# arendu-zz/MacaronicUserModeling

Hardware: AMD Instinct MI355X
Metric: LBP sweep iters/sec (whole node), batch=8192 graphs |X|=64 (higher is better)
Workload: dtype f64

## Files before the change

### macaronicusermodeling_amd/csrc/mlbp_lean.hip

```cpp
#include <hip/hip_runtime.h>

#include <vector>

#include "mlbp_device.h"
#include "mlbp_internal.h"

using mlbp::fail;
using namespace mlbp_dev;

namespace {

constexpr int WG = 256;

typedef double nt_d2 __attribute__((ext_vector_type(2)));
#define NT_LOAD2(p) ([&] { const nt_d2 v_ = __builtin_nontemporal_load(reinterpret_cast<const nt_d2*>(p)); return make_double2(v_.x, v_.y); }())

constexpr int GROUP_WORDS = 48;
using mlbp::UOP_VAR; using mlbp::UOP_MT; using mlbp::UOP_PSLOT_SHIFT; using mlbp::UOP_NOP; using mlbp::UOP_STORE_VF;
using mlbp::UOP_NSRC_SHIFT; using mlbp::UOP_CARRY_IN; using mlbp::UOP_CARRY_OUT;

struct LeanDev {
  const int32_t* image;
  const int32_t* readout;
  uint8_t* bail;
  int32_t n_bundles, HL, n_cprod, WL, n_ext, init, dense, keep;
};

__device__ __forceinline__ double swapadd16(double a, double b) {
  auto lo = __builtin_amdgcn_permlane16_swap((unsigned)__double2loint(a), (unsigned)__double2loint(b), false, false);
  auto hi = __builtin_amdgcn_permlane16_swap((unsigned)__double2hiint(a), (unsigned)__double2hiint(b), false, false);
  return __hiloint2double((int)hi[0], (int)lo[0]) + __hiloint2double((int)hi[1], (int)lo[1]);
}
__device__ __forceinline__ double swapadd32(double a, double b) {
  auto lo = __builtin_amdgcn_permlane32_swap((unsigned)__double2loint(a), (unsigned)__double2loint(b), false, false);
  auto hi = __builtin_amdgcn_permlane32_swap((unsigned)__double2hiint(a), (unsigned)__double2hiint(b), false, false);
  return __hiloint2double((int)hi[0], (int)lo[0]) + __hiloint2double((int)hi[1], (int)lo[1]);
}

__device__ __forceinline__ bool vote_any(bool p, int32_t* votes, int wave, int lane) {
  const int mine = __ballot(p) != 0 ? 1 : 0;
  if (lane == 0) votes[wave] = mine;
  lds_barrier();
  const int4 v = *reinterpret_cast<const int4*>(votes);
  return (v.x | v.y | v.z | v.w) != 0;
}

struct LaneGeo {
  int tm0, tm1;
  int mt;
  int red_tm;
  int red_mt;
  bool up, st_tm, st_mt, wr_tm;
};

__device__ __forceinline__ double2 lds2(const char* p) { return *reinterpret_cast<const double2*>(p); }
__device__ __forceinline__ void mul2(double2& a, const double2 b) { a.x *= b.x; a.y *= b.y; }

struct RegTable {
  const double2 (&T)[4][2];
  __device__ __forceinline__ double2 operator()(int r, int k) const { return T[r][k]; }
};
struct LdsTable {
  const double2* base;
  __device__ __forceinline__ double2 operator()(int r, int k) const { return base[(r * 2 + k) * WG]; }
};

template <bool MT, bool WIDE, typename TB>
__device__ __forceinline__ void contract(const TB T, char* wb, int u0, int s1, int s2, int s3, int s4, int vf,
                                         const LaneGeo& G, char* redA) {
  const int nsrc = (u0 >> UOP_NSRC_SHIFT) & 15;
  const bool has_vf = (u0 & UOP_STORE_VF) != 0;
  if (MT) {
    double2 ma = lds2(wb + s1 + G.mt), mb = lds2(wb + s1 + G.mt + 16);
    {
      const double2 a = lds2(wb + s2 + G.mt), b = lds2(wb + s2 + G.mt + 16);
      mul2(ma, a); mul2(mb, b);
    }
    if (nsrc > 2) {
      if (WIDE) {
        const double2 a2 = lds2(wb + s3 + G.mt), b2 = lds2(wb + s3 + G.mt + 16);
        const double2 a3 = lds2(wb + s4 + G.mt), b3 = lds2(wb + s4 + G.mt + 16);
        mul2(ma, a2); mul2(mb, b2);
        mul2(ma, a3); mul2(mb, b3);
      } else {
        mul2(ma, lds2(wb + s3 + G.mt)); mul2(mb, lds2(wb + s3 + G.mt + 16));
        if (nsrc > 3) { mul2(ma, lds2(wb + s4 + G.mt)); mul2(mb, lds2(wb + s4 + G.mt + 16)); }
      }
    }
    if (has_vf && G.st_mt) {
      *reinterpret_cast<double2*>(wb + vf + G.mt) = ma;
      *reinterpret_cast<double2*>(wb + vf + G.mt + 16) = mb;
    }
    double a00, a01, a10, a11;
    { const double2 t0 = T(0, 0), t1 = T(0, 1); a00 = ma.x * t0.x; a01 = ma.x * t0.y; a10 = ma.x * t1.x; a11 = ma.x * t1.y; }
    { const double2 t0 = T(1, 0), t1 = T(1, 1); a00 += ma.y * t0.x; a01 += ma.y * t0.y; a10 += ma.y * t1.x; a11 += ma.y * t1.y; }
    { const double2 t0 = T(2, 0), t1 = T(2, 1); a00 += mb.x * t0.x; a01 += mb.x * t0.y; a10 += mb.x * t1.x; a11 += mb.x * t1.y; }
    { const double2 t0 = T(3, 0), t1 = T(3, 1); a00 += mb.y * t0.x; a01 += mb.y * t0.y; a10 += mb.y * t1.x; a11 += mb.y * t1.y; }
    a00 += dpp_mov<0x128>(a10);
    a01 += dpp_mov<0x128>(a11);
    *reinterpret_cast<double*>(redA + G.red_mt) = swapadd32(a00, a01);
  } else {
    double2 m0 = lds2(wb + s1 + G.tm0), m1 = lds2(wb + s1 + G.tm1);
    {
      const double2 a = lds2(wb + s2 + G.tm0), b = lds2(wb + s2 + G.tm1);
      mul2(m0, a); mul2(m1, b);
    }
    if (nsrc > 2) {
      if (WIDE) {
        const double2 a2 = lds2(wb + s3 + G.tm0), b2 = lds2(wb + s3 + G.tm1);
        const double2 a3 = lds2(wb + s4 + G.tm0), b3 = lds2(wb + s4 + G.tm1);
        mul2(m0, a2); mul2(m1, b2);
        mul2(m0, a3); mul2(m1, b3);
      } else {
        mul2(m0, lds2(wb + s3 + G.tm0)); mul2(m1, lds2(wb + s3 + G.tm1));
        if (nsrc > 3) { mul2(m0, lds2(wb + s4 + G.tm0)); mul2(m1, lds2(wb + s4 + G.tm1)); }
      }
    }
    if (has_vf && G.st_tm) {
      *reinterpret_cast<double2*>(wb + vf + G.tm0) = m0;
      *reinterpret_cast<double2*>(wb + vf + G.tm1) = m1;
    }
    double v[4];
#pragma unroll
    for (int r = 0; r < 4; ++r) {
      const double2 t0 = T(r, 0), t1 = T(r, 1);
      v[r] = t0.x * m0.x;
      v[r] += t0.y * m0.y;
      v[r] += t1.x * m1.x;
      v[r] += t1.y * m1.y;
    }
    const double u0 = swapadd16(v[0], v[2]), u1 = swapadd16(v[1], v[3]);
    const double keep = G.up ? u1 : u0, send = G.up ? u0 : u1;
    double w = keep + dpp_mov<0x141>(send);
    w += dpp_mov<0xB1>(w);
    w += dpp_mov<0x4E>(w);
    *reinterpret_cast<double*>(redA + G.red_tm) = w;
  }
}

template <int NT, int NL>
__device__ __forceinline__ void front(const double2 (&tab)[NT][4][2], const double2* tl, char* wb, int u0, const int4& lo, const int4& hi,
                                      const LaneGeo& G, char* redA) {
  const int pslot = (u0 >> UOP_PSLOT_SHIFT) & 7;
#pragma unroll
  for (int p = 0; p < NT; ++p) {
    if (p == pslot) {
      if (u0 & UOP_MT) contract<true, (NT > 1)>(RegTable{tab[p]}, wb, u0, lo.y, lo.z, lo.w, hi.x, hi.y, G, redA);
      else contract<false, (NT > 1)>(RegTable{tab[p]}, wb, u0, lo.y, lo.z, lo.w, hi.x, hi.y, G, redA);
    }
  }
  if (NL > 0 && pslot >= NT) {
    const LdsTable T = {tl + (size_t)(pslot - NT) * 8 * WG};
    if (u0 & UOP_MT) contract<true, (NT > 1)>(T, wb, u0, lo.y, lo.z, lo.w, hi.x, hi.y, G, redA);
    else contract<false, (NT > 1)>(T, wb, u0, lo.y, lo.z, lo.w, hi.x, hi.y, G, redA);
  }
}

struct Src { double2 a, b; };

__device__ __forceinline__ void gather_pair(char* wb, int uA, const int4& A0, const int4& A1, int uB, const int4& B0, const int4& B1,
                                            const LaneGeo& G, Src& mA, Src& mB) {
  const bool mtA = (uA & UOP_MT) != 0, mtB = (uB & UOP_MT) != 0;
  const int a0 = mtA ? G.mt : G.tm0, a1 = mtA ? G.mt + 16 : G.tm1;
  const int b0 = mtB ? G.mt : G.tm0, b1 = mtB ? G.mt + 16 : G.tm1;
  mA.a = lds2(wb + A0.y + a0); mA.b = lds2(wb + A0.y + a1);
  mB.a = lds2(wb + B0.y + b0); mB.b = lds2(wb + B0.y + b1);
  {
    const double2 pa = lds2(wb + A0.z + a0), pb = lds2(wb + A0.z + a1);
    const double2 qa = lds2(wb + B0.z + b0), qb = lds2(wb + B0.z + b1);
    mul2(mA.a, pa); mul2(mA.b, pb);
    mul2(mB.a, qa); mul2(mB.b, qb);
  }
  if (((uA >> UOP_NSRC_SHIFT) & 15) > 2) {
    const double2 pa = lds2(wb + A0.w + a0), pb = lds2(wb + A0.w + a1);
    const double2 ra = lds2(wb + A1.x + a0), rb = lds2(wb + A1.x + a1);
    mul2(mA.a, pa); mul2(mA.b, pb);
    mul2(mA.a, ra); mul2(mA.b, rb);
  }
  if (((uB >> UOP_NSRC_SHIFT) & 15) > 2) {
    const double2 qa = lds2(wb + B0.w + b0), qb = lds2(wb + B0.w + b1);
    const double2 sa = lds2(wb + B1.x + b0), sb = lds2(wb + B1.x + b1);
    mul2(mB.a, qa); mul2(mB.b, qb);
    mul2(mB.a, sa); mul2(mB.b, sb);
  }
  if ((uA & UOP_STORE_VF) && (mtA ? G.st_mt : G.st_tm)) {
    *reinterpret_cast<double2*>(wb + A1.y + a0) = mA.a;
    *reinterpret_cast<double2*>(wb + A1.y + a1) = mA.b;
  }
  if ((uB & UOP_STORE_VF) && (mtB ? G.st_mt : G.st_tm)) {
    *reinterpret_cast<double2*>(wb + B1.y + b0) = mB.a;
    *reinterpret_cast<double2*>(wb + B1.y + b1) = mB.b;
  }
}

template <bool MT, typename TB>
__device__ __forceinline__ void contract_gathered(const TB T, const Src m, const LaneGeo& G, char* redA) {
#pragma clang fp contract(off)
  if (MT) {
    const double2 ma = m.a, mb = m.b;
    double a00, a01, a10, a11;
    { const double2 t0 = T(1, 0), t1 = T(1, 1); a00 = ma.y * t0.x; a01 = ma.y * t0.y; a10 = ma.y * t1.x; a11 = ma.y * t1.y; }
#define MLBP_ROW(mv, r) { const double2 t0 = T(r, 0), t1 = T(r, 1); a00 = __builtin_fma(mv, t0.x, a00); a01 = __builtin_fma(mv, t0.y, a01); \
                          a10 = __builtin_fma(mv, t1.x, a10); a11 = __builtin_fma(mv, t1.y, a11); }
    MLBP_ROW(ma.x, 0)
    MLBP_ROW(mb.x, 2)
    MLBP_ROW(mb.y, 3)
#undef MLBP_ROW
    a00 += dpp_mov<0x128>(a10);
    a01 += dpp_mov<0x128>(a11);
    *reinterpret_cast<double*>(redA + G.red_mt) = swapadd32(a00, a01);
  } else {
    const double2 m0 = m.a, m1 = m.b;
    double v[4];
#pragma unroll
    for (int r = 0; r < 4; ++r) {
      const double2 t0 = T(r, 0), t1 = T(r, 1);
      v[r] = t0.y * m0.y;
      v[r] = __builtin_fma(t0.x, m0.x, v[r]);
      v[r] = __builtin_fma(t1.x, m1.x, v[r]);
      v[r] = __builtin_fma(t1.y, m1.y, v[r]);
    }
    const double u0 = swapadd16(v[0], v[2]), u1 = swapadd16(v[1], v[3]);
    const double keep = G.up ? u1 : u0, send = G.up ? u0 : u1;
    double w = keep + dpp_mov<0x141>(send);
    w += dpp_mov<0xB1>(w);
    w += dpp_mov<0x4E>(w);
    *reinterpret_cast<double*>(redA + G.red_tm) = w;
  }
}

template <int NT>
__device__ __forceinline__ void front_gathered(const double2 (&tab)[NT][4][2], int u0, const Src m, const LaneGeo& G, char* redA) {
  const int pslot = (u0 >> UOP_PSLOT_SHIFT) & 7;
#pragma unroll
  for (int p = 0; p < NT; ++p) {
    if (p == pslot) {
      if (u0 & UOP_MT) contract_gathered<true>(RegTable{tab[p]}, m, G, redA);
      else contract_gathered<false>(RegTable{tab[p]}, m, G, redA);
    }
  }
}

template <int NT>
__device__ __forceinline__ void gradient_epilogue(const SweepDev& d, const GradFusedDev& gf, const double2 (&tab)[NT][4][2],
                                                  const char* wb, const int32_t* gst, double* scratch, const LaneGeo& G, int g,
                                                  int R_, int c_, int b3_) {
  constexpr int FEE = 3, FED = 6;
  const int t = threadIdx.x, lane = t & 63, wave = __builtin_amdgcn_readfirstlane(t >> 6);
  double lf[FEE] = {0.0, 0.0, 0.0};
  bool lbad = false;
  if (t < NT && t < d.P) {
    const int l0 = gf.pair_label[((size_t)g * d.P + t) * 2], l1 = gf.pair_label[((size_t)g * d.P + t) * 2 + 1];
    if ((unsigned)l0 >= 64u || (unsigned)l1 >= 64u) lbad = true;
    else {
      const double* phl = (gf.pair_phi[t] ? gf.phi_en_en_w1 : gf.phi_en_en) + ((size_t)l0 * 64 + l1) * FEE;
#pragma unroll
      for (int q = 0; q < FEE; ++q) lf[q] = phl[q];
    }
  }
  int which = 0;
  double2 W[NT][4][2];
  double* zs = scratch + 512;
  double* lfs = scratch + 544;
#pragma unroll
  for (int p = 0; p < NT; ++p) {
    double z = 0.0;
    if (p < d.P) {
      const int cs = as_const(gf.pair_c_slot)[p], rs = as_const(gf.pair_r_slot)[p];
      which |= (as_const(gf.pair_phi)[p] ? 1 : 0) << p;
      const double2 ca = lds2(wb + cs * 512 + G.mt), cb = lds2(wb + cs * 512 + G.mt + 16);
      const double2 r0 = lds2(wb + rs * 512 + G.tm0), r1 = lds2(wb + rs * 512 + G.tm1);
#pragma unroll
      for (int r = 0; r < 4; ++r) {
        const double ci = r == 0 ? ca.x : (r == 1 ? ca.y : (r == 2 ? cb.x : cb.y));
#pragma unroll
        for (int k = 0; k < 2; ++k) {
          const double2 rj = k ? r1 : r0, T = tab[p][r][k];
          W[p][r][k] = make_double2((ci * rj.x) * T.x, (ci * rj.y) * T.y);
          z += W[p][r][k].x + W[p][r][k].y;
        }
      }
      z = wave_sum(z);
      if (lane == 0) zs[wave * NT + p] = z;
    } else {
#pragma unroll
      for (int r = 0; r < 4; ++r) W[p][r][0] = W[p][r][1] = make_double2(0.0, 0.0);
    }
  }
  if (lbad) atomicExch(d.status, 1);
  if (t < NT && t < d.P) {
#pragma unroll
    for (int q = 0; q < FEE; ++q) lfs[t * FEE + q] = lf[q];
  }
  lds_barrier();
  double2 V[2][4][2];
#pragma unroll
  for (int tz = 0; tz < 2; ++tz)
#pragma unroll
    for (int r = 0; r < 4; ++r) V[tz][r][0] = V[tz][r][1] = make_double2(0.0, 0.0);
#pragma unroll
  for (int p = 0; p < NT; ++p) {
    if (p < d.P) {
      const double Z = (zs[p] + zs[NT + p]) + (zs[2 * NT + p] + zs[3 * NT + p]);
      const double inv = Z > 0.0 ? 1.0 / Z : 0.0;
      const double i0 = ((which >> p) & 1) ? 0.0 : inv, i1 = ((which >> p) & 1) ? inv : 0.0;
#pragma unroll
      for (int r = 0; r < 4; ++r)
#pragma unroll
        for (int k = 0; k < 2; ++k) {
          V[0][r][k].x += W[p][r][k].x * i0; V[0][r][k].y += W[p][r][k].y * i0;
          V[1][r][k].x += W[p][r][k].x * i1; V[1][r][k].y += W[p][r][k].y * i1;
        }
    }
  }
  double gacc[2][FEE] = {{0.0, 0.0, 0.0}, {0.0, 0.0, 0.0}};
  const int all = (1 << (d.P < NT ? d.P : NT)) - 1;
#pragma unroll
  for (int tz = 0; tz < 2; ++tz) {
    if (tz ? (which & all) == 0 : (which & all) == all) continue;
    typedef double v2d __attribute__((ext_vector_type(2)));
    typedef const v2d __attribute__((address_space(1))) * gptr2;
    const double* phi = tz ? gf.phi_en_en_w1 : gf.phi_en_en;
#pragma unroll
    for (int k = 0; k < 2; ++k) {
      const int col = 32 * (k ? 1 - b3_ : b3_) + 2 * c_;
      v2d cell[4][3];
#pragma unroll
      for (int r = 0; r < 4; ++r) {
        const gptr2 ph = (gptr2)(uintptr_t)(phi + ((size_t)(4 * R_ + r) * 64 + col) * FEE);
        cell[r][0] = ph[0]; cell[r][1] = ph[1]; cell[r][2] = ph[2];
      }
#pragma unroll
      for (int r = 0; r < 4; ++r) {
        const double w0 = V[tz][r][k].x, w1 = V[tz][r][k].y;
        gacc[tz][0] += w0 * cell[r][0].x + w1 * cell[r][1].y;
        gacc[tz][1] += w0 * cell[r][0].y + w1 * cell[r][2].x;
        gacc[tz][2] += w0 * cell[r][1].x + w1 * cell[r][2].y;
      }
    }
  }
  double gsum[FEE];
#pragma unroll
  for (int q = 0; q < FEE; ++q) gsum[q] = wave_sum(gacc[0][q] + gacc[1][q]);
  double lab_ee[FEE] = {0.0, 0.0, 0.0}, lab_ed[FED] = {0.0, 0.0, 0.0, 0.0, 0.0, 0.0};
  double exp_ee[FEE] = {0.0, 0.0, 0.0}, exp_ed[FED] = {0.0, 0.0, 0.0, 0.0, 0.0, 0.0};
  bool bad = false;
  constexpr int UB = 6;
  const int U = d.U;
  for (int u0 = wave; u0 < U; u0 += 4 * UB) {
    double b[UB], pv[UB][FED];
    int kd[UB], at[UB];
#pragma unroll
    for (int j = 0; j < UB; ++j) {
      const int u = u0 + 4 * j;
      kd[j] = -1;
      if (u < U) {
        const int kind = __builtin_amdgcn_readfirstlane(gst[2 * U + u]), obs = __builtin_amdgcn_readfirstlane(gst[3 * U + u]);
        const int lab = __builtin_amdgcn_readfirstlane(gst[4 * U + u]);
        const int cols = kind == 2 ? gf.Vde : 64;
        if ((unsigned)obs >= (unsigned)cols || (unsigned)lab >= 64u || (unsigned)kind > 2u) { bad = true; continue; }
        kd[j] = kind;
        const int slot = __builtin_amdgcn_readfirstlane(gst[u]);
        b[j] = __builtin_amdgcn_readfirstlane(gst[U + u]) ? *reinterpret_cast<const double*>(wb + slot * 512 + lane * 8) : 0.0;
        if (kind == 2) {
          const double2* ph = reinterpret_cast<const double2*>(gf.phi_en_de_t + ((size_t)obs * 64 + lane) * FED);
          at[j] = (obs * 64 + lab) * FED;
          const double2 a0 = ph[0], a1 = ph[1], a2 = ph[2];
          pv[j][0] = a0.x; pv[j][1] = a0.y; pv[j][2] = a1.x; pv[j][3] = a1.y; pv[j][4] = a2.x; pv[j][5] = a2.y;
        } else {
          typedef const double __attribute__((address_space(1))) * gptr1;
          const gptr1 ph = (gptr1)(uintptr_t)((kind ? gf.phi_en_en_w1_t : gf.phi_en_en_t) + ((size_t)obs * 64 + lane) * FEE);
          at[j] = (obs * 64 + lab) * FEE;
#pragma unroll
          for (int q = 0; q < FEE; ++q) pv[j][q] = ph[q];
        }
      }
    }
#pragma unroll
    for (int j = 0; j < UB; ++j) {
      if (kd[j] == 2) {
#pragma unroll
        for (int q = 0; q < FED; ++q) { lab_ed[q] += as_const_f64(gf.phi_en_de_t)[at[j] + q]; exp_ed[q] += b[j] * pv[j][q]; }
      } else if (kd[j] >= 0) {
        const double* base = kd[j] ? gf.phi_en_en_w1_t : gf.phi_en_en_t;
#pragma unroll
        for (int q = 0; q < FEE; ++q) { lab_ee[q] += as_const_f64(base)[at[j] + q]; exp_ee[q] += b[j] * pv[j][q]; }
      }
    }
  }
  if (bad && lane == 0) atomicExch(d.status, 1);
  constexpr int PER = FEE + FEE + FED;
  {
    double ue[FEE], ud[FED];
#pragma unroll
    for (int q = 0; q < FEE; ++q) ue[q] = lab_ee[q] - wave_sum(exp_ee[q]);
#pragma unroll
    for (int q = 0; q < FED; ++q) ud[q] = lab_ed[q] - wave_sum(exp_ed[q]);
    if (lane == 0) {
      double* o = scratch + wave * PER;
#pragma unroll
      for (int q = 0; q < FEE; ++q) o[q] = gsum[q];
#pragma unroll
      for (int q = 0; q < FEE; ++q) o[FEE + q] = ue[q];
#pragma unroll
      for (int q = 0; q < FED; ++q) o[FEE + FEE + q] = ud[q];
    }
  }
  lds_barrier();
  if (t == 0) {
    double tot[PER];
#pragma unroll
    for (int q = 0; q < PER; ++q) tot[q] = (scratch[q] + scratch[PER + q]) + (scratch[2 * PER + q] + scratch[3 * PER + q]);
    double gee[FEE];
#pragma unroll
    for (int q = 0; q < FEE; ++q) gee[q] = tot[FEE + q] - tot[q];
#pragma unroll
    for (int p = 0; p < NT; ++p) {
      if (p < d.P) {
#pragma unroll
        for (int q = 0; q < FEE; ++q) gee[q] += lfs[p * FEE + q];
      }
    }
#pragma unroll
    for (int q = 0; q < FEE; ++q) gf.grad_en_en[(size_t)g * FEE + q] = gee[q];
#pragma unroll
    for (int q = 0; q < FED; ++q) gf.grad_en_de[(size_t)g * FED + q] = tot[FEE + FEE + q];
  }
}

__device__ __forceinline__ double rescale(double r, int& bad) {
  const unsigned key = mag_key(r);
  const unsigned long long normal = __ballot(key - KEY_MIN < KEY_BAD - KEY_MIN);
  const unsigned long long wrong = __ballot(key >= KEY_BAD);
  bad |= (wrong != 0) | (normal == 0);
  const int ref = __builtin_amdgcn_readlane((int)key, normal ? __builtin_ctzll(normal) : 0);
  return __builtin_ldexp(r, 1023 - ((ref >> 20) & 0x7FF));
}

template <int NT, bool PADX, bool MULTI, int NL, bool GRAD>
__global__ __launch_bounds__(WG, (NT >= 7 ? 1 : (NT >= 4 ? 2 : 3))) void sweep_x64_lean_kernel(SweepDev d, LeanDev f, const int32_t* groups,
                                                                                             int n_groups, GradFusedDev gf) {
  int g = blockIdx.x;
  if (MULTI) {
    int lo = 0, hi = n_groups - 1;
    while (lo < hi) {
      const int mid = (lo + hi + 1) >> 1;
      if (as_const(groups)[(size_t)mid * GROUP_WORDS] <= g) lo = mid; else hi = mid - 1;
    }
    const int32_t* G = groups + (size_t)lo * GROUP_WORDS;
    const Words16 w0 = sload16(G), w1 = sload16(G + 16), w2 = sload16(G + 32);
    auto ptr = [](int32_t a, int32_t b) { return (uintptr_t)(uint32_t)a | ((uintptr_t)(uint32_t)b << 32); };
    g -= w0.w[0];
    f.image = (const int32_t*)ptr(w0.w[2], w0.w[3]); f.readout = (const int32_t*)ptr(w0.w[4], w0.w[5]);
    f.bail = (uint8_t*)ptr(w0.w[6], w0.w[7]); d.msgs = (double*)ptr(w0.w[8], w0.w[9]);
    d.marginals = (double*)ptr(w0.w[10], w0.w[11]); d.pair_tables = (const double*)ptr(w0.w[12], w0.w[13]);
    d.pair_tab = (const int32_t*)ptr(w0.w[14], w0.w[15]); d.unary_tables = (const double*)ptr(w1.w[0], w1.w[1]);
    d.unary_tab = (const int32_t*)ptr(w1.w[2], w1.w[3]); d.status = (int32_t*)ptr(w1.w[4], w1.w[5]);
    f.n_bundles = w1.w[6]; f.HL = w1.w[7]; f.n_cprod = w1.w[8]; f.WL = w1.w[9]; f.n_ext = w1.w[10];
    d.n_msgs = w1.w[11]; d.P = w1.w[12]; d.U = w1.w[13]; d.n_vars = w1.w[14]; d.n_pair_tables = w1.w[15];
    d.n_unary_tables = w2.w[0]; f.dense = w2.w[1];
  }
  extern __shared__ double lds[];
  double* work = lds;
  double* red = lds + (size_t)(d.n_msgs + f.n_ext) * 64;
  int32_t* limg = reinterpret_cast<int32_t*>(red + 4 * 256);
  double2* tl = reinterpret_cast<double2*>(limg + 16 * (f.n_bundles + 1));
  int32_t* gst = reinterpret_cast<int32_t*>(tl + (size_t)NL * 8 * WG);

  const int t = threadIdx.x, lane = t & 63, wave = __builtin_amdgcn_readfirstlane(t >> 6);
  const int X = PADX ? d.X : 64;
  const double uniform = 1.0 / (double)X;
  const double uni_l = (!PADX || lane < X) ? uniform : 0.0;
  double* gm = d.msgs + (size_t)g * d.n_msgs * X;
  const int32_t* img_hoist = f.image + 16 * (size_t)f.n_bundles;
  const int32_t* img_cprod = img_hoist + 8 * (size_t)f.HL;
  const int32_t* img_written = img_cprod + 16 * (size_t)f.n_cprod;
  int32_t* votes = reinterpret_cast<int32_t*>(red);
  constexpr bool LEAN_SYNC = !GRAD;
  constexpr bool EARLY = !GRAD;
  constexpr bool PAIR_GATHER = !GRAD && NL == 0 && NT == 3;
  static_assert(!(GRAD && PADX), "the GRAD form of phase A loads whole rows: X = 64 only");

  LaneGeo G;
  const int c_ = (lane & 7) | ((lane >> 1) & 8), b3_ = (lane >> 3) & 1, R_ = 4 * wave + (b3_ | ((lane >> 5) << 1));
  {
    const int b5 = lane >> 5, b4 = (lane >> 4) & 1, b2 = (lane >> 2) & 1;
    G.tm0 = (32 * b3_ + 2 * c_) * 8;
    G.tm1 = (32 * (1 - b3_) + 2 * c_) * 8;
    G.mt = 4 * R_ * 8;
    G.red_tm = (4 * R_ + 2 * b4 + b2) * 8;
    G.red_mt = (wave * 64 + 32 * b3_ + 2 * c_ + b5) * 8;
    G.up = b2 != 0;
    G.st_tm = wave == 0 && (lane & 0x28) == 0;
    G.st_mt = (lane & 0x17) == 0;
    G.wr_tm = (lane & 3) == 0;
  }

  if (t == 0) f.bail[g] = 0;
  int g_kind = 0, g_obs = 0, g_lab = 0;
  if (GRAD && t < d.U) {
    g_kind = gf.unary_kind[t]; g_obs = gf.unary_obs[(size_t)g * d.U + t]; g_lab = gf.unary_label[(size_t)g * d.U + t];
  }
  bool ok = true;
  const double* nowhere = reinterpret_cast<const double*>(f.image);
  constexpr int HB = 8;
  double ur[HB];
  int uslot[HB], ufac[HB];
  {
    const Words16 hl = sload16(img_hoist + wave * 2 * f.HL);
#pragma unroll
    for (int j = 0; j < HB; ++j) {
      const int u = hl.w[2 * j];
      uslot[j] = hl.w[2 * j + 1];
      ufac[j] = u;
      if (EARLY) {
        int row = -1;
        if (u >= 0) row = f.dense ? g * d.U + u : as_const(d.unary_tab)[(size_t)g * d.U + u];
        const bool in = (unsigned)row < (unsigned)d.n_unary_tables;
        if (u >= 0 && !in) ok = false;
        const double* at = in ? d.unary_tables + (size_t)row * X + (PADX ? min(lane, X - 1) : lane) : nowhere;
        ur[j] = *at;
      } else {
        ur[j] = 0.0;
        if (u >= 0) {
          const int row = f.dense ? g * d.U + u : as_const(d.unary_tab)[(size_t)g * d.U + u];
          if ((unsigned)row >= (unsigned)d.n_unary_tables) ok = false;
          else ur[j] = d.unary_tables[(size_t)row * X + lane];
        }
      }
    }
  }
  double2 tab[NT][4][2];
#pragma unroll
  for (int p = 0; p < NT; ++p) {
    if (!PADX && EARLY) {
      const int pc = p < d.P ? p : 0;
      const int ti = f.dense ? g * d.P + pc : as_const(d.pair_tab)[(size_t)g * d.P + pc];
      const bool in = (unsigned)ti < (unsigned)d.n_pair_tables;
      if (p < d.P && !in) ok = false;
      const double* T = (p < d.P && in) ? d.pair_tables + (size_t)ti * 4096 + (size_t)(4 * R_) * 64 + 2 * c_ : nowhere;
#pragma unroll
      for (int r = 0; r < 4; ++r) {
        tab[p][r][0] = NT_LOAD2(T + r * 64 + 32 * b3_);
        tab[p][r][1] = NT_LOAD2(T + r * 64 + 32 * (1 - b3_));
      }
    } else if (p < d.P) {
      const int ti = f.dense ? g * d.P + p : as_const(d.pair_tab)[(size_t)g * d.P + p];
      if ((unsigned)ti >= (unsigned)d.n_pair_tables) { ok = false; continue; }
      if (!PADX) {
        const double* T = d.pair_tables + (size_t)ti * 4096 + (size_t)(4 * R_) * 64 + 2 * c_;
#pragma unroll
        for (int r = 0; r < 4; ++r) {
          tab[p][r][0] = NT_LOAD2(T + r * 64 + 32 * b3_);
          tab[p][r][1] = NT_LOAD2(T + r * 64 + 32 * (1 - b3_));
        }
      } else {
        const double* T = d.pair_tables + (size_t)ti * X * X;
#pragma unroll
        for (int r = 0; r < 4; ++r)
#pragma unroll
          for (int k = 0; k < 2; ++k) {
            const int row = 4 * R_ + r, col = 32 * (k ? 1 - b3_ : b3_) + 2 * c_;
            tab[p][r][k].x = (row < X && col < X) ? T[(size_t)row * X + col] : 0.0;
            tab[p][r][k].y = (row < X && col + 1 < X) ? T[(size_t)row * X + col + 1] : 0.0;
          }
      }
    }
  }
#pragma unroll
  for (int p = NT; p < NT + NL; ++p) {
    if (p < d.P && !PADX) {
      const int ti = f.dense ? g * d.P + p : as_const(d.pair_tab)[(size_t)g * d.P + p];
      if ((unsigned)ti >= (unsigned)d.n_pair_tables) { ok = false; continue; }
      const double* T = d.pair_tables + (size_t)ti * 4096 + (size_t)(4 * R_) * 64 + 2 * c_;
#pragma unroll
      for (int r = 0; r < 4; ++r)
#pragma unroll
        for (int k = 0; k < 2; ++k) {
          typedef __attribute__((address_space(3))) void* lds_ptr;
          typedef const __attribute__((address_space(1))) void* glb_ptr;
          double2* dst = tl + ((p - NT) * 8 + r * 2 + k) * WG + wave * 64;
          __builtin_amdgcn_global_load_lds((glb_ptr)(T + r * 64 + 32 * (k ? 1 - b3_ : b3_)), (lds_ptr)dst, 16, 0, 0);
        }
    }
  }
  int dense_word = 0;
  bool dense_ok = true;
  if (EARLY) {
    const int i = min(t, d.P + d.U - 1);
    const int32_t* at = i < d.P ? d.pair_tab + (size_t)g * d.P + i : d.unary_tab + (size_t)g * d.U + (i - d.P);
    dense_word = *(f.dense ? at : f.image);
  } else if (f.dense) {
    for (int i = t; i < d.P + d.U; i += WG)
      dense_ok &= i < d.P ? d.pair_tab[(size_t)g * d.P + i] == g * d.P + i : d.unary_tab[(size_t)g * d.U + (i - d.P)] == g * d.U + (i - d.P);
  }
  constexpr int PW = 2;
  int32_t pre[PW];
#pragma unroll
  for (int q = 0; q < PW; ++q)
    pre[q] = EARLY ? f.image[min(t + q * WG, 16 * (f.n_bundles + 1) - 1)] : ((t + q * WG < 16 * (f.n_bundles + 1)) ? f.image[t + q * WG] : 0);
  unsigned bad_key = 0;
  {
    double2* dst = reinterpret_cast<double2*>(work);
    const int x0 = (2 * t) & 63;
    const double2 uni2 = PADX ? make_double2(x0 < X ? uniform : 0.0, x0 + 1 < X ? uniform : 0.0) : make_double2(uniform, uniform);
    if (f.init) {
      for (int i = t; i < d.n_msgs * 32; i += WG) dst[i] = uni2;
    } else if (!PADX) {
      const double2* src = reinterpret_cast<const double2*>(gm);
      for (int i = t; i < d.n_msgs * 32; i += WG) {
        const double2 v = src[i];
        bad_key = max(bad_key, max(mag_key(v.x), mag_key(v.y)));
        dst[i] = v;
      }
    } else {
      for (int i = t; i < d.n_msgs * 64; i += WG) {
        const int slot = i >> 6, x = i & 63;
        const double v = x < X ? gm[(size_t)slot * X + x] : 0.0;
        bad_key = max(bad_key, mag_key(v));
        work[i] = v;
      }
    }
    if (t < 32) dst[d.n_msgs * 32 + t] = uni2;
    if (t >= 32 && t < 64) dst[(d.n_msgs + f.n_ext - 1) * 32 + (t - 32)] = make_double2(1.0, 1.0);
  }
  lds_barrier();
#pragma unroll
  for (int j = 0; j < HB; ++j) {
    if (uslot[j] >= 0) {
      const double r = (!PADX || lane < X) ? ur[j] : 0.0;
      const double s = wave_sum(r);
      const double m = renorm(r, s, uni_l, true);
      bad_key = max(bad_key, s > 0.0 ? mag_key(m) : KEY_BAD);
      work[uslot[j] * 64 + lane] = m;
      if (GRAD && lane == 0) { gst[ufac[j]] = uslot[j]; gst[d.U + ufac[j]] = s > 0.0 ? 1 : 0; }
    }
  }
  if (GRAD && t < d.U) { gst[2 * d.U + t] = g_kind; gst[3 * d.U + t] = g_obs; gst[4 * d.U + t] = g_lab; }
  for (int j = HB; j < f.HL; ++j) {
    const const_i32p hp = as_const(img_hoist + (wave * f.HL + j) * 2);
    const int u = hp[0], slot = hp[1];
    if (u < 0) break;
    const int row = f.dense ? g * d.U + u : as_const(d.unary_tab)[(size_t)g * d.U + u];
    double r = 0.0;
    if ((unsigned)row >= (unsigned)d.n_unary_tables) ok = false;
    else if (!PADX || lane < X) r = d.unary_tables[(size_t)row * X + lane];
    const double s = wave_sum(r);
    const double m = renorm(r, s, uni_l, true);
    bad_key = max(bad_key, s > 0.0 ? mag_key(m) : KEY_BAD);
    work[slot * 64 + lane] = m;
    if (GRAD && lane == 0) { gst[u] = slot; gst[d.U + u] = s > 0.0 ? 1 : 0; }
  }
  if (LEAN_SYNC ? vote_any(!ok, votes, wave, lane) : !__syncthreads_and(ok ? 1 : 0)) {
    if (t == 0) atomicExch(d.status, 1);
    if (f.init)
      for (int i = t; i < d.n_msgs * X; i += WG) gm[i] = uniform;
    return;
  }
  for (int k = wave; k < f.n_cprod; k += 4) {
    const Words16 cl = sload16(img_cprod + 16 * k);
    double acc = uni_l;
#pragma unroll
    for (int q0 = 1; q0 < 16; q0 += 5) {
      if (cl.w[0] >= q0) {
        double m[5];
#pragma unroll
        for (int q = 0; q < 5; ++q) m[q] = work[cl.w[q0 + q] * 64 + lane];
#pragma unroll
        for (int q = 0; q < 5; ++q) acc *= m[q];
      }
    }
    bad_key = max(bad_key, mag_key(acc));
    work[(d.n_msgs + 1 + k) * 64 + lane] = acc;
  }
  auto fill_limg = [&]() {
    if (NL > 0) asm volatile("s_waitcnt vmcnt(0)" ::: "memory");
#pragma unroll
    for (int q = 0; q < PW; ++q)
      if (t + q * WG < 16 * (f.n_bundles + 1)) limg[t + q * WG] = pre[q];
    for (int i = t + PW * WG; i < 16 * (f.n_bundles + 1); i += WG) limg[i] = f.image[i];
  };
  if (LEAN_SYNC) fill_limg();
  if (LEAN_SYNC ? vote_any(bad_key >= KEY_BAD, votes + 1024, wave, lane) : __syncthreads_or(bad_key >= KEY_BAD ? 1 : 0) != 0) {
    if (t == 0) f.bail[g] = 1;
    return;
  }
  if (!LEAN_SYNC) { fill_limg(); lds_barrier(); }

  char* wb = reinterpret_cast<char*>(work);
  int parity = 0, bad = 0;
  double carry = 1.0;
  const int4* li = reinterpret_cast<const int4*>(limg);
  int4 A0 = li[0], A1 = li[1], B0 = li[2], B1 = li[3];
  for (int k = 0; k < f.n_bundles; ++k) {
    int4 nA0, nA1, nB0, nB1;
#define MLBP_FETCH_NEXT() (nA0 = li[4 * k + 4], nA1 = li[4 * k + 5], nB0 = li[4 * k + 6], nB1 = li[4 * k + 7])
    if (!PAIR_GATHER) MLBP_FETCH_NEXT();
    const int fA = __builtin_amdgcn_readfirstlane(A0.x), fB = __builtin_amdgcn_readfirstlane(B0.x);
    if (fA & UOP_VAR) {
      if (PAIR_GATHER) MLBP_FETCH_NEXT();
      const int nsrc = (fA >> UOP_NSRC_SHIFT) & 15;
      double m = work[(A0.y >> 3) + lane];
      const double m2 = work[(A0.z >> 3) + lane];
      if (fA & UOP_CARRY_IN) m *= carry;
      m *= m2;
      if (nsrc > 2) {
        const double m3 = work[(A0.w >> 3) + lane], m4 = work[(A1.x >> 3) + lane];
        m *= m3;
        m *= m4;
      }
      if (fA & UOP_CARRY_OUT) carry = m;
      else work[(A1.y >> 3) + lane] = m;
    } else {
      char* redP = reinterpret_cast<char*>(red) + parity * 4096;
      const bool two = !(fB & UOP_NOP);
      if (PAIR_GATHER) {
        Src mA, mB;
        gather_pair(wb, fA, A0, A1, fB, B0, B1, G, mA, mB);
        MLBP_FETCH_NEXT();
        front_gathered<NT>(tab, fA, mA, G, redP);
        if (two) front_gathered<NT>(tab, fB, mB, G, redP + 2048);
      } else {
        front<NT, NL>(tab, tl + t, wb, fA, A0, A1, G, redP);
        if (two) front<NT, NL>(tab, tl + t, wb, fB, B0, B1, G, redP + 2048);
      }
      lds_barrier();
      const double* rd = reinterpret_cast<const double*>(redP);
      double rA = rd[lane];
      if (fA & UOP_MT) rA = (rA + rd[64 + lane]) + (rd[128 + lane] + rd[192 + lane]);
      work[(A1.z >> 3) + lane] = rescale(rA, bad);
      if (two) {
        double rB = rd[256 + lane];
        if (fB & UOP_MT) rB = (rB + rd[320 + lane]) + (rd[384 + lane] + rd[448 + lane]);
        work[(B1.z >> 3) + lane] = rescale(rB, bad);
      }
      parity ^= 1;
    }
    A0 = nA0; A1 = nA1; B0 = nB0; B1 = nB1;
#undef MLBP_FETCH_NEXT
  }
  if (bad) {
    if (t == 0) f.bail[g] = 2;
    return;
  }
  lds_barrier();
  double marg[2] = {0.0, 0.0};
  if (EARLY) dense_ok = !f.dense || t >= d.P + d.U || dense_word == (t < d.P ? g * d.P + t : g * d.U + (t - d.P));
  bool bad_out = !dense_ok;
  if (f.readout) {
#pragma unroll
    for (int j = 0; j < 2; ++j) {
      const int v = wave + 4 * j;
      if (v < d.n_vars) {
        const Words16 rl = sload16(f.readout + 16 * v);
        double acc = work[rl.w[1] * 64 + lane];
#pragma unroll
        for (int q0 = 2; q0 < 16; q0 += 7) {
          if (rl.w[0] >= q0) {
            double m[7];
#pragma unroll
            for (int q = 0; q < 7; ++q) m[q] = work[rl.w[q0 + q] * 64 + lane];
#pragma unroll
            for (int q = 0; q < 7; ++q) acc *= m[q];
          }
        }
        const unsigned key = wave_max_u32(mag_key(acc));
        bad_out |= key >= KEY_BAD || key < KEY_MIN;
        marg[j] = acc / wave_sum(acc);
      }
    }
    for (int v = wave + 8; v < d.n_vars; v += 4) {
      const Words16 rl = sload16(f.readout + 16 * v);
      double acc = work[rl.w[1] * 64 + lane];
      for (int q = 2; q <= rl.w[0]; ++q) acc *= work[as_const(f.readout + 16 * v)[q] * 64 + lane];
      const unsigned key = wave_max_u32(mag_key(acc));
      bad_out |= key >= KEY_BAD || key < KEY_MIN;
      if (!bad_out) d.marginals[((size_t)g * d.n_vars + v) * 64 + lane] = acc / wave_sum(acc);
    }
  }
  lds_barrier();
  if (f.keep || GRAD) {
    for (int j0 = 0; j0 < f.WL; j0 += 4) {
      const const_i32p wl = as_const(img_written + wave * f.WL + j0);
      int slot[4];
      double v[4], s[4];
#pragma unroll
      for (int j = 0; j < 4; ++j) { slot[j] = wl[j]; v[j] = slot[j] >= 0 ? work[slot[j] * 64 + lane] : 1.0; }
#pragma unroll
      for (int j = 0; j < 4; ++j) {
        const unsigned key = wave_max_u32(mag_key(v[j]));
        bad_out |= key >= KEY_BAD || key < KEY_MIN;
        s[j] = wave_sum(v[j]);
      }
#pragma unroll
      for (int j = 0; j < 4; ++j)
        if (slot[j] >= 0) work[slot[j] * 64 + lane] = v[j] / s[j];
    }
  }
  if (LEAN_SYNC ? vote_any(bad_out, votes, wave, lane) : __syncthreads_or(bad_out ? 1 : 0) != 0) {
    if (t == 0) f.bail[g] = 3;
    return;
  }
  if (f.keep && !PADX) {
    const double2* src = reinterpret_cast<const double2*>(work);
    double2* dst = reinterpret_cast<double2*>(gm);
    for (int i = t; i < d.n_msgs * 32; i += WG) dst[i] = src[i];
  } else if (f.keep) {
    for (int i = t; i < d.n_msgs * 64; i += WG)
      if ((i & 63) < X) gm[(size_t)(i >> 6) * X + (i & 63)] = work[i];
  }
  if (f.readout) {
#pragma unroll
    for (int j = 0; j < 2; ++j) {
      const int v = wave + 4 * j;
      if (v < d.n_vars) d.marginals[((size_t)g * d.n_vars + v) * 64 + lane] = marg[j];
    }
  }
  if (GRAD) {
    gradient_epilogue<NT>(d, gf, tab, reinterpret_cast<const char*>(work), gst, reinterpret_cast<double*>(red), G, g, R_, c_, b3_);
  }
}

}

namespace mlbp {

static int lean_plan(mlbp_program* prog, const mlbp_sweep_args* a, bool grad, bool* ok, SweepDev* d, LeanDev* f, size_t* lds) {
  *ok = false;
  const LeanProgram& lp = prog->lean;
  if (!lp.ok || !prog->d_limage || a->X > 64 || a->X < 2 || !a->normalize_messages || prog->P < 1 || prog->P > 8) return MLBP_OK;
  const bool padx = a->X < 64;
  if (padx && prog->P > 4) return MLBP_OK;
  if (a->gradient && padx) return MLBP_OK;
  if (grad && (prog->P > 3 || prog->U > WG)) return fail(MLBP_EINVAL, "lean kernel: fused gradient needs P <= 3 and U <= %d", WG);
  if (a->flags & MLBP_SWEEP_APPROX_INFERENCE) return MLBP_OK;
  if (a->marginals && !prog->d_lreadout && !padx) return MLBP_OK;
  const int n_ext = 2 + lp.n_cprod;
  *lds = ((size_t)(prog->n_msgs + n_ext) * 64 + 4 * 256) * sizeof(double) + 16 * (size_t)(lp.n_bundles + 1) * sizeof(int32_t);
  if (prog->P == 7 && !padx) *lds += 32 * 1024;
  if (grad) *lds += 5 * (size_t)prog->U * sizeof(int32_t);
  if (*lds > 80 * 1024) return MLBP_OK;
  if (prog->P + prog->U > WG) return MLBP_OK;
  const bool dense = (a->flags & MLBP_SWEEP_DENSE_TABLES) != 0;
  if (dense && ((int64_t)a->B * prog->P > a->n_pair_tables || (int64_t)a->B * prog->U > a->n_unary_tables))
    return fail(MLBP_EINVAL, "mlbp_sweep_f64: MLBP_SWEEP_DENSE_TABLES needs B*P pair tables and B*U unary columns");
  if (prog->d_bail.bytes < (size_t)a->B)
    if (int e = mlbp_program_reserve(prog, a->B)) return e;
  d->pair_tables = a->pair_tables; d->pair_tab = a->pair_tab;
  d->unary_tables = a->unary_tables; d->unary_tab = a->unary_tab;
  d->msgs = a->msgs;
  d->ops = nullptr; d->srcs = nullptr; d->sweeps = nullptr; d->pairseq = nullptr;
  d->status = prog->d_status;
  d->n_sweeps = prog->n_sweeps; d->n_msgs = prog->n_msgs; d->P = prog->P; d->U = prog->U; d->X = a->X;
  d->n_pair_tables = a->n_pair_tables; d->n_unary_tables = a->n_unary_tables;
  d->marginals = padx ? nullptr : a->marginals; d->readout = nullptr; d->n_vars = prog->n_vars;
  d->only = nullptr; d->fill_uniform = 0; d->approx_k = 0;
  f->image = prog->d_limage; f->readout = (a->marginals && !padx) ? prog->d_lreadout : nullptr; f->bail = prog->d_bail;
  f->n_bundles = lp.n_bundles; f->HL = lp.HL; f->n_cprod = lp.n_cprod; f->WL = lp.WL;
  f->n_ext = n_ext; f->init = a->init_messages; f->dense = dense ? 1 : 0;
  const bool waived = (a->flags & MLBP_SWEEP_NO_MESSAGE_WRITEBACK) && !padx && (a->marginals || grad) && (!a->gradient || grad);
  f->keep = waived ? 0 : 1;
  *ok = true;
  return MLBP_OK;
}

typedef void (*lean_fn)(SweepDev, LeanDev, const int32_t*, int, GradFusedDev);

template <bool MULTI>
static lean_fn pick_lean(int P, bool padx) {
  if constexpr (!MULTI) {
    if (padx) {
      switch (P) {
        case 1: return sweep_x64_lean_kernel<1, true, false, 0, false>;
        case 2: return sweep_x64_lean_kernel<2, true, false, 0, false>;
        case 3: return sweep_x64_lean_kernel<3, true, false, 0, false>;
        default: return sweep_x64_lean_kernel<4, true, false, 0, false>;
      }
    }
  }
  switch (P) {
    case 1: return sweep_x64_lean_kernel<1, false, MULTI, 0, false>;
    case 2: return sweep_x64_lean_kernel<2, false, MULTI, 0, false>;
    case 3: return sweep_x64_lean_kernel<3, false, MULTI, 0, false>;
    case 4: return sweep_x64_lean_kernel<4, false, MULTI, 0, false>;
    case 5: case 6: return sweep_x64_lean_kernel<6, false, MULTI, 0, false>;
    case 7: return sweep_x64_lean_kernel<6, false, MULTI, 1, false>;
    default: return sweep_x64_lean_kernel<8, false, MULTI, 0, false>;
  }
}
static lean_fn pick_lean_grad(int P) {
  switch (P) {
    case 1: return sweep_x64_lean_kernel<1, false, false, 0, true>;
    case 2: return sweep_x64_lean_kernel<2, false, false, 0, true>;
    default: return sweep_x64_lean_kernel<3, false, false, 0, true>;
  }
}

int launch_lean_sweep(mlbp_program* prog, const mlbp_sweep_args* a, bool fuse_gradient, void* stream, bool* launched) {
  *launched = false;
  SweepDev d;
  LeanDev f;
  size_t lds = 0;
  bool ok = false;
  if (int e = lean_plan(prog, a, fuse_gradient, &ok, &d, &f, &lds)) return e;
  if (!ok) return MLBP_OK;
  GradFusedDev gf = {};
  if (fuse_gradient) fill_grad_fused(a->gradient, &gf);
  lean_fn k = fuse_gradient ? pick_lean_grad(prog->P) : pick_lean<false>(prog->P, a->X < 64);
  if (int e = grant_lds((const void*)k, lds)) return e;
  launch_begin();
  MLBP_LAUNCH(k, dim3(a->B), dim3(WG), lds, (hipStream_t)stream, d, f, nullptr, 0, gf);
  if (int e = launch_verdict("lean sweep")) return e;
  *launched = true;
  return MLBP_OK;
}

int launch_lean_groups(mlbp_program* const* progs, const mlbp_sweep_args* args, int n_groups, void* stream, std::vector<char>& member) {
  std::vector<int32_t> table;
  size_t lds_max = 0;
  int p_max = 0, total = 0, n_in = 0;
  SweepDev d0;
  LeanDev f0;
  for (int k = 0; k < n_groups; ++k) {
    if (!member[k]) continue;
    member[k] = 0;
    if (args[k].X != 64) continue;
    SweepDev d;
    LeanDev f;
    size_t lds = 0;
    bool ok = false;
    if (int e = lean_plan(progs[k], &args[k], false, &ok, &d, &f, &lds)) return e;
    if (!ok) continue;
    if (n_in == 0) { d0 = d; f0 = f; }
    else if (f.init != f0.init || f.keep != f0.keep || (f.readout != nullptr) != (f0.readout != nullptr)) continue;
    member[k] = 1;
    ++n_in;
    lds_max = std::max(lds_max, lds + (progs[k]->P < 7 ? 32 * 1024 : 0));
    p_max = std::max(p_max, (int)progs[k]->P);
    table.resize(table.size() + GROUP_WORDS, 0);
    int32_t* w = &table[table.size() - GROUP_WORDS];
    auto put = [&](int at, const void* p) { const uintptr_t v = (uintptr_t)p; w[at] = (int32_t)(uint32_t)v; w[at + 1] = (int32_t)(uint32_t)(v >> 32); };
    w[0] = total; w[1] = args[k].B;
    put(2, f.image); put(4, f.readout); put(6, f.bail); put(8, d.msgs); put(10, d.marginals); put(12, d.pair_tables);
    put(14, d.pair_tab); put(16, d.unary_tables); put(18, d.unary_tab); put(20, d.status);
    w[22] = f.n_bundles; w[23] = f.HL; w[24] = f.n_cprod; w[25] = f.WL; w[26] = f.n_ext; w[27] = d.n_msgs; w[28] = d.P; w[29] = d.U;
    w[30] = d.n_vars; w[31] = d.n_pair_tables; w[32] = d.n_unary_tables; w[33] = f.dense;
    total += args[k].B;
  }
  if (n_in == 0) return MLBP_OK;
  int32_t* d_gtable = nullptr;
  if (int e = group_table_device(progs[0]->gtables, table, stream, &d_gtable)) return e;
  lean_fn k = pick_lean<true>(p_max, false);
  if (int e = grant_lds((const void*)k, lds_max)) return e;
  launch_begin();
  MLBP_LAUNCH(k, dim3(total), dim3(WG), lds_max, (hipStream_t)stream, d0, f0, d_gtable, n_in, GradFusedDev{});
  return launch_verdict("grouped lean sweep");
}

}
```

Before: 14340.

## Use raw LDS addresses, branch-split stores, and defer rescale bad-check to loop end

For the pair-gather path, LDS accesses now use precomputed 32-bit address-space-3 offsets, with the work base folded into the lane geometry, so the generic-pointer address arithmetic goes away. The VF store predicate is recomputed from threadIdx with a scalar branch guard. Per-rescale ballot checks for bad keys are replaced by a running max and min that yield a single verdict after the loop. This cuts per-bundle scalar and vector instruction overhead, but adds code paths and some register pressure.

```diff
diff --git a/macaronicusermodeling_amd/csrc/mlbp_lean.hip b/macaronicusermodeling_amd/csrc/mlbp_lean.hip
--- a/macaronicusermodeling_amd/csrc/mlbp_lean.hip
+++ b/macaronicusermodeling_amd/csrc/mlbp_lean.hip
@@ -55,6 +55,19 @@
 
 __device__ __forceinline__ double2 lds2(const char* p) { return *reinterpret_cast<const double2*>(p); }
 __device__ __forceinline__ void mul2(double2& a, const double2 b) { a.x *= b.x; a.y *= b.y; }
+
+typedef double lds_v2d __attribute__((ext_vector_type(2)));
+__device__ __forceinline__ int lds_addr(const void* p) { return (int)(size_t)(const __attribute__((address_space(3))) char*)p; }
+__device__ __forceinline__ double2 lds2_at(int a) {
+  const lds_v2d v = *(const __attribute__((address_space(3))) lds_v2d*)(size_t)(unsigned)a;
+  return make_double2(v.x, v.y);
+}
+__device__ __forceinline__ void lds2_put(int a, const double2 v) {
+  lds_v2d w; w.x = v.x; w.y = v.y;
+  *(__attribute__((address_space(3))) lds_v2d*)(size_t)(unsigned)a = w;
+}
+__device__ __forceinline__ double lds1_at(int a) { return *(const __attribute__((address_space(3))) double*)(size_t)(unsigned)a; }
+__device__ __forceinline__ void lds1_put(int a, double v) { *(__attribute__((address_space(3))) double*)(size_t)(unsigned)a = v; }
 
 struct RegTable {
   const double2 (&T)[4][2];
@@ -158,39 +171,49 @@
 
 struct Src { double2 a, b; };
 
+template <bool STORE_BRANCH, bool LDS_ADDR>
 __device__ __forceinline__ void gather_pair(char* wb, int uA, const int4& A0, const int4& A1, int uB, const int4& B0, const int4& B1,
                                             const LaneGeo& G, Src& mA, Src& mB) {
   const bool mtA = (uA & UOP_MT) != 0, mtB = (uB & UOP_MT) != 0;
   const int a0 = mtA ? G.mt : G.tm0, a1 = mtA ? G.mt + 16 : G.tm1;
   const int b0 = mtB ? G.mt : G.tm0, b1 = mtB ? G.mt + 16 : G.tm1;
-  mA.a = lds2(wb + A0.y + a0); mA.b = lds2(wb + A0.y + a1);
-  mB.a = lds2(wb + B0.y + b0); mB.b = lds2(wb + B0.y + b1);
+  auto rd = [&](int off) { return LDS_ADDR ? lds2_at(off) : lds2(wb + off); };
+  auto wr = [&](int off, const double2 v) { if (LDS_ADDR) lds2_put(off, v); else *reinterpret_cast<double2*>(wb + off) = v; };
+  mA.a = rd(A0.y + a0); mA.b = rd(A0.y + a1);
+  mB.a = rd(B0.y + b0); mB.b = rd(B0.y + b1);
   {
-    const double2 pa = lds2(wb + A0.z + a0), pb = lds2(wb + A0.z + a1);
-    const double2 qa = lds2(wb + B0.z + b0), qb = lds2(wb + B0.z + b1);
+    const double2 pa = rd(A0.z + a0), pb = rd(A0.z + a1);
+    const double2 qa = rd(B0.z + b0), qb = rd(B0.z + b1);
     mul2(mA.a, pa); mul2(mA.b, pb);
     mul2(mB.a, qa); mul2(mB.b, qb);
   }
   if (((uA >> UOP_NSRC_SHIFT) & 15) > 2) {
-    const double2 pa = lds2(wb + A0.w + a0), pb = lds2(wb + A0.w + a1);
-    const double2 ra = lds2(wb + A1.x + a0), rb = lds2(wb + A1.x + a1);
+    const double2 pa = rd(A0.w + a0), pb = rd(A0.w + a1);
+    const double2 ra = rd(A1.x + a0), rb = rd(A1.x + a1);
     mul2(mA.a, pa); mul2(mA.b, pb);
     mul2(mA.a, ra); mul2(mA.b, rb);
   }
   if (((uB >> UOP_NSRC_SHIFT) & 15) > 2) {
-    const double2 qa = lds2(wb + B0.w + b0), qb = lds2(wb + B0.w + b1);
-    const double2 sa = lds2(wb + B1.x + b0), sb = lds2(wb + B1.x + b1);
+    const double2 qa = rd(B0.w + b0), qb = rd(B0.w + b1);
+    const double2 sa = rd(B1.x + b0), sb = rd(B1.x + b1);
     mul2(mB.a, qa); mul2(mB.b, qb);
     mul2(mB.a, sa); mul2(mB.b, sb);
   }
-  if ((uA & UOP_STORE_VF) && (mtA ? G.st_mt : G.st_tm)) {
-    *reinterpret_cast<double2*>(wb + A1.y + a0) = mA.a;
-    *reinterpret_cast<double2*>(wb + A1.y + a1) = mA.b;
-  }
-  if ((uB & UOP_STORE_VF) && (mtB ? G.st_mt : G.st_tm)) {
-    *reinterpret_cast<double2*>(wb + B1.y + b0) = mB.a;
-    *reinterpret_cast<double2*>(wb + B1.y + b1) = mB.b;
-  }
+  if (STORE_BRANCH) {
+    const int t = threadIdx.x;
+    auto mine = [&](bool mt) { return (t & (mt ? 0x17 : 0xE8)) == 0; };
+    if (uA & UOP_STORE_VF) {
+      asm volatile("");
+      if (mine(mtA)) { wr(A1.y + a0, mA.a); wr(A1.y + a1, mA.b); }
+    }
+    if (uB & UOP_STORE_VF) {
+      asm volatile("");
+      if (mine(mtB)) { wr(B1.y + b0, mB.a); wr(B1.y + b1, mB.b); }
+    }
+    return;
+  }
+  if ((uA & UOP_STORE_VF) && (mtA ? G.st_mt : G.st_tm)) { wr(A1.y + a0, mA.a); wr(A1.y + a1, mA.b); }
+  if ((uB & UOP_STORE_VF) && (mtB ? G.st_mt : G.st_tm)) { wr(B1.y + b0, mB.a); wr(B1.y + b1, mB.b); }
 }
 
 template <bool MT, typename TB>
@@ -437,6 +460,15 @@
   return __builtin_ldexp(r, 1023 - ((ref >> 20) & 0x7FF));
 }
 
+__device__ __forceinline__ double rescale_kmax(double r, unsigned& some, unsigned& kmax) {
+  const unsigned key = mag_key(r);
+  const unsigned long long normal = __ballot(key - KEY_MIN < KEY_BAD - KEY_MIN);
+  kmax = max(kmax, key);
+  some = min(some, (unsigned)normal | (unsigned)(normal >> 32));
+  const int ref = __builtin_amdgcn_readlane((int)key, normal ? __builtin_ctzll(normal) : 0);
+  return __builtin_ldexp(r, 1023 - ((ref >> 20) & 0x7FF));
+}
+
 template <int NT, bool PADX, bool MULTI, int NL, bool GRAD>
 __global__ __launch_bounds__(WG, (NT >= 7 ? 1 : (NT >= 4 ? 2 : 3))) void sweep_x64_lean_kernel(SweepDev d, LeanDev f, const int32_t* groups,
                                                                                              int n_groups, GradFusedDev gf) {
@@ -479,6 +511,9 @@
   constexpr bool LEAN_SYNC = !GRAD;
   constexpr bool EARLY = !GRAD;
   constexpr bool PAIR_GATHER = !GRAD && NL == 0 && NT == 3;
+  constexpr bool STORE_BRANCH = PAIR_GATHER;
+  constexpr bool ONE_VERDICT = PAIR_GATHER;
+  constexpr bool LDS_ADDR = PAIR_GATHER;
   static_assert(!(GRAD && PADX), "the GRAD form of phase A loads whole rows: X = 64 only");
 
   LaneGeo G;
@@ -494,7 +529,9 @@
     G.st_tm = wave == 0 && (lane & 0x28) == 0;
     G.st_mt = (lane & 0x17) == 0;
     G.wr_tm = (lane & 3) == 0;
-  }
+    if (LDS_ADDR) { const int base = lds_addr(work); G.tm0 += base; G.tm1 += base; G.mt += base; }
+  }
+  const int lane8 = LDS_ADDR ? lds_addr(work) + lane * 8 : 0;
 
   if (t == 0) f.bail[g] = 0;
   int g_kind = 0, g_obs = 0, g_lab = 0;
@@ -689,6 +726,7 @@
 
   char* wb = reinterpret_cast<char*>(work);
   int parity = 0, bad = 0;
+  unsigned kmax = 0, some = ~0u;
   double carry = 1.0;
   const int4* li = reinterpret_cast<const int4*>(limg);
   int4 A0 = li[0], A1 = li[1], B0 = li[2], B1 = li[3];
@@ -700,23 +738,25 @@
     if (fA & UOP_VAR) {
       if (PAIR_GATHER) MLBP_FETCH_NEXT();
       const int nsrc = (fA >> UOP_NSRC_SHIFT) & 15;
-      double m = work[(A0.y >> 3) + lane];
-      const double m2 = work[(A0.z >> 3) + lane];
+      double m = LDS_ADDR ? lds1_at(A0.y + lane8) : work[(A0.y >> 3) + lane];
+      const double m2 = LDS_ADDR ? lds1_at(A0.z + lane8) : work[(A0.z >> 3) + lane];
       if (fA & UOP_CARRY_IN) m *= carry;
       m *= m2;
       if (nsrc > 2) {
-        const double m3 = work[(A0.w >> 3) + lane], m4 = work[(A1.x >> 3) + lane];
+        const double m3 = LDS_ADDR ? lds1_at(A0.w + lane8) : work[(A0.w >> 3) + lane];
+        const double m4 = LDS_ADDR ? lds1_at(A1.x + lane8) : work[(A1.x >> 3) + lane];
         m *= m3;
         m *= m4;
       }
       if (fA & UOP_CARRY_OUT) carry = m;
+      else if (LDS_ADDR) lds1_put(A1.y + lane8, m);
       else work[(A1.y >> 3) + lane] = m;
     } else {
       char* redP = reinterpret_cast<char*>(red) + parity * 4096;
       const bool two = !(fB & UOP_NOP);
       if (PAIR_GATHER) {
         Src mA, mB;
-        gather_pair(wb, fA, A0, A1, fB, B0, B1, G, mA, mB);
+        gather_pair<STORE_BRANCH, LDS_ADDR>(wb, fA, A0, A1, fB, B0, B1, G, mA, mB);
         MLBP_FETCH_NEXT();
         front_gathered<NT>(tab, fA, mA, G, redP);
         if (two) front_gathered<NT>(tab, fB, mB, G, redP + 2048);
@@ -728,17 +768,20 @@
       const double* rd = reinterpret_cast<const double*>(redP);
       double rA = rd[lane];
       if (fA & UOP_MT) rA = (rA + rd[64 + lane]) + (rd[128 + lane] + rd[192 + lane]);
-      work[(A1.z >> 3) + lane] = rescale(rA, bad);
+      if (LDS_ADDR) lds1_put(A1.z + lane8, ONE_VERDICT ? rescale_kmax(rA, some, kmax) : rescale(rA, bad));
+      else work[(A1.z >> 3) + lane] = ONE_VERDICT ? rescale_kmax(rA, some, kmax) : rescale(rA, bad);
       if (two) {
         double rB = rd[256 + lane];
         if (fB & UOP_MT) rB = (rB + rd[320 + lane]) + (rd[384 + lane] + rd[448 + lane]);
-        work[(B1.z >> 3) + lane] = rescale(rB, bad);
+        if (LDS_ADDR) lds1_put(B1.z + lane8, ONE_VERDICT ? rescale_kmax(rB, some, kmax) : rescale(rB, bad));
+        else work[(B1.z >> 3) + lane] = ONE_VERDICT ? rescale_kmax(rB, some, kmax) : rescale(rB, bad);
       }
       parity ^= 1;
     }
     A0 = nA0; A1 = nA1; B0 = nB0; B1 = nB1;
 #undef MLBP_FETCH_NEXT
   }
+  if (ONE_VERDICT) bad = some == 0 || __ballot(kmax >= KEY_BAD) != 0;
   if (bad) {
     if (t == 0) f.bail[g] = 2;
     return;
```

New measurement: 14590 (median of 6 runs). 1.02x the previous value.
